# Hi-FT/ERD

Measured on AMD Instinct MI355X. Metric: images/sec GFL-R50 40+40 incre step @1333x800, higher is better.
Workload: dtype f32; 1 GPU; gfl_r50_fpn first_40_incre_last_40 ERD (BASELINE configs[1]), 1333x800 padded to 800x1344, fp32, procedural weights; batch_per_gpu=4, global_batch=4, parallelism=dp1

## Files before the change

### erd_amd/csrc/conv_mfma.hip

```cpp
#include <algorithm>
#include <type_traits>
#include "erd_common.h"
#include <stdlib.h>
#ifndef ERD_SGB
#define ERD_SGB 0
#endif

namespace {

typedef float f32x16 __attribute__((ext_vector_type(16)));
typedef __bf16 bf16x8 __attribute__((ext_vector_type(8)));
typedef __bf16 bf16x2v __attribute__((ext_vector_type(2)));
typedef float f32x2v __attribute__((ext_vector_type(2)));

__device__ __forceinline__ float pack_bf16(float a, float b) {
    const f32x2v v = {a, b};
    return __builtin_bit_cast(float, __builtin_convertvector(v, bf16x2v));
}

constexpr int NTHREADS = 256;

#ifdef ERD_IGEMM_TRACE
constexpr int IG_NS = 32;
__device__ unsigned long long g_igemm_trace[1024 * IG_NS];
// ... 1650 lines not shown
        int s = 0;
        for (; s + 3 < nsplit; s += 4) {
            const float4 v0 = *reinterpret_cast<const float4*>(part + (s + 0) * slab + o);
            const float4 v1 = *reinterpret_cast<const float4*>(part + (s + 1) * slab + o);
            const float4 v2 = *reinterpret_cast<const float4*>(part + (s + 2) * slab + o);
            const float4 v3 = *reinterpret_cast<const float4*>(part + (s + 3) * slab + o);
            g.x += (v0.x + v1.x) + (v2.x + v3.x); g.y += (v0.y + v1.y) + (v2.y + v3.y);
            g.z += (v0.z + v1.z) + (v2.z + v3.z); g.w += (v0.w + v1.w) + (v2.w + v3.w);
        }
        for (; s < nsplit; ++s) {
            const float4 v = *reinterpret_cast<const float4*>(part + s * slab + o);
            g.x += v.x; g.y += v.y; g.z += v.z; g.w += v.w;
        }
        if (rowdot) {
            const float4 ww = *reinterpret_cast<const float4*>(w + o);
            dot = ww.x * g.x + ww.y * g.y + ww.z * g.z + ww.w * g.w;
        }
        float4 o4 = make_float4(rs * g.x, rs * g.y, rs * g.z, rs * g.w);
        if (accumulate) {
            const float4 old = *reinterpret_cast<const float4*>(dW + o);
            o4.x += old.x; o4.y += old.y; o4.z += old.z; o4.w += old.w;
        }
        *reinterpret_cast<float4*>(dW + o) = o4;
    }
    if (rowdot) {
        __shared__ float red[4];
        dot = erd::wave_sum(dot);
        if ((threadIdx.x & 63) == 0) red[threadIdx.x >> 6] = dot;
        __syncthreads();
        if (threadIdx.x == 0) atomicAdd(rowdot + co, red[0] + red[1] + red[2] + red[3]);
    }
}

template <typename OutT>
__global__ __launch_bounds__(256) void weight_transpose_kernel(const float* __restrict__ w,
                                                                const float* __restrict__ rowscale,
                                                                OutT* __restrict__ dst, int Cout, int ntaps, int Cin,
                                                                int flip) {
    __shared__ float tile[32][33];
    const int t = blockIdx.z;
    const int td = flip ? ntaps - 1 - t : t;
    const int ci0 = blockIdx.x * 32, co0 = blockIdx.y * 32;
    const int tx = threadIdx.x & 31, ty = threadIdx.x >> 5;
    for (int r = ty; r < 32; r += 8) {
        const int co = co0 + r, ci = ci0 + tx;
        float v = 0.f;
        if (co < Cout && ci < Cin) v = w[((int64_t)co * ntaps + t) * Cin + ci] * (rowscale ? rowscale[co] : 1.f);
        tile[r][tx] = v;
    }
    __syncthreads();
    for (int r = ty; r < 32; r += 8) {
        const int ci = ci0 + r, co = co0 + tx;
        if (co < Cout && ci < Cin) dst[((int64_t)ci * ntaps + td) * Cout + co] = (OutT)tile[tx][r];
    }
}

using erd::limbs3;

__global__ __launch_bounds__(256) void split3_kernel(const float* __restrict__ src, unsigned short* __restrict__ dst, int64_t n) {
    const int64_t i = blockIdx.x * 256ll + threadIdx.x;
    if (i >= n) return;
    unsigned short h, m, l;
    limbs3(src[i], h, m, l);
    dst[i] = h;
    dst[n + i] = m;
    dst[2 * n + i] = l;
}

__global__ __launch_bounds__(256) void weight_transpose_x3_kernel(const float* __restrict__ w, const float* __restrict__ rowscale,
                                                                   unsigned short* __restrict__ dst, int Cout, int ntaps, int Cin,
                                                                   int flip) {
    __shared__ float tile[32][33];
    const int t = blockIdx.z;
    const int td = flip ? ntaps - 1 - t : t;
    const int ci0 = blockIdx.x * 32, co0 = blockIdx.y * 32;
    const int tx = threadIdx.x & 31, ty = threadIdx.x >> 5;
    for (int r = ty; r < 32; r += 8) {
        const int co = co0 + r, ci = ci0 + tx;
        float v = 0.f;
        if (co < Cout && ci < Cin) v = w[((int64_t)co * ntaps + t) * Cin + ci] * (rowscale ? rowscale[co] : 1.f);
        tile[r][tx] = v;
    }
    __syncthreads();
    const int64_t plane = (int64_t)Cin * ntaps * Cout;
    for (int r = ty; r < 32; r += 8) {
        const int ci = ci0 + r, co = co0 + tx;
        if (co < Cout && ci < Cin) {
            unsigned short h, m, l;
            limbs3(tile[tx][r], h, m, l);
            const int64_t o = ((int64_t)ci * ntaps + td) * Cout + co;
            dst[o] = h;
            dst[plane + o] = m;
            dst[2 * plane + o] = l;
        }
    }
}

int num_cus() {
    static int n = 0;
    if (n == 0) {
        int dev = 0;
        hipDeviceProp_t prop;
        if (hipGetDevice(&dev) == hipSuccess && hipGetDeviceProperties(&prop, dev) == hipSuccess)
            n = prop.multiProcessorCount;
        if (n <= 0) n = 256;
    }
    return n;
}

struct IgemmShape { int64_t mtiles; bool seg_taps; };

int igemm_plan(const erd_conv_desc* d, const IgemmShape& sh, int tiles, int nkt, int BKT, int MINW, bool BF, SkWs& ws) {
    const int slots = MINW * erd::usable_cus(num_cus());
    int G = tiles;
    ws = SkWs{nullptr, nullptr, xcd_order_enabled(), 0};
    const size_t slab_bytes = (size_t)2 * 4 * num_cus() * 128 * 128 * sizeof(float);
    const size_t need = slab_bytes + (size_t)tiles * sizeof(int);
    const bool ragged = tiles < 8 * slots && (tiles % slots) != 0;
    const bool sk_pays = BF ? tiles * 2 <= slots : true;
    static const int min_slices = getenv("ERD_SK_MIN_SLICES") ? atoi(getenv("ERD_SK_MIN_SLICES")) : 8;
    const int64_t units = (int64_t)tiles * nkt;
    const bool tiny = units < slots && min_slices > 0 && nkt >= 2 * min_slices && !BF;
    if (sh.seg_taps) ws.xcd_order = 0;
    static const int sk_min_k = getenv("ERD_SK_MIN_K") ? atoi(getenv("ERD_SK_MIN_K")) : 512;
    if (d->sk_ws && d->sk_ws_bytes >= need && ragged && sk_pays && !sh.seg_taps && nkt * BKT >= sk_min_k && (units >= slots || tiny)) {
        G = (int)std::min<int64_t>(slots, min_slices > 0 ? std::max<int64_t>(tiles, units / min_slices) : slots);
        ws.slabs = reinterpret_cast<float*>(d->sk_ws);
        ws.cnt = reinterpret_cast<int*>(reinterpret_cast<char*>(d->sk_ws) + slab_bytes);
// ... 231 lines not shown
    if (rowdot && !(accumulate & 2)) (void)hipMemsetAsync(rowdot, 0, sizeof(float) * Cout, (hipStream_t)stream);
    hipLaunchKernelGGL(wgrad_reduce_kernel, dim3(Cout, (K + 1023) / 1024), dim3(256), 0, (hipStream_t)stream, part,
                       nsplit, Cout, K, w, rowscale, dW, accumulate & 1, rowdot, erd_wgrad_reduce_groups{});
    return erd::check_launch("wgrad_reduce");
}

extern "C" int erd_wgrad_reduce_grouped(const float* part, int nsplit, int Cout, int K, const erd_wgrad_reduce_groups* groups,
                                        int accumulate, erd_stream_t stream) {
    ERD_REQUIRE(part && groups && nsplit >= 1 && Cout >= 1 && K >= 4 && K % 4 == 0, "wgrad_reduce_grouped: bad args");
    ERD_REQUIRE(groups->ngroups >= 1 && groups->ngroups <= ERD_MAX_GROUPS, "wgrad_reduce_grouped: ngroups=%d", groups->ngroups);
    for (int g = 0; g < groups->ngroups; ++g) {
        ERD_REQUIRE(groups->dW[g], "wgrad_reduce_grouped: group %d has no dW", g);
        ERD_REQUIRE(!groups->rowdot[g] || groups->w[g], "wgrad_reduce_grouped: rowdot of group %d needs w", g);
    }
    if (!(accumulate & 2))
        for (int g = 0; g < groups->ngroups; ++g)
            if (groups->rowdot[g]) (void)hipMemsetAsync(groups->rowdot[g], 0, sizeof(float) * Cout, (hipStream_t)stream);
    hipLaunchKernelGGL(wgrad_reduce_kernel, dim3(Cout, (K + 1023) / 1024, groups->ngroups), dim3(256), 0, (hipStream_t)stream, part,
                       nsplit, Cout, K, nullptr, nullptr, nullptr, accumulate & 1, nullptr, *groups);
    return erd::check_launch("wgrad_reduce_grouped");
}

extern "C" int erd_wgrad_reduce_rows(const float* part, int nsplit, int Cout_slab, int Cout, int K, float* dW,
                                     int accumulate, erd_stream_t stream) {
    ERD_REQUIRE(part && dW && nsplit >= 1 && K % 4 == 0 && Cout >= 1 && Cout <= Cout_slab, "wgrad_reduce_rows: bad args");
    hipLaunchKernelGGL(wgrad_reduce_kernel, dim3(Cout, (K + 1023) / 1024), dim3(256), 0, (hipStream_t)stream, part,
                       nsplit, Cout_slab, K, nullptr, nullptr, dW, accumulate & 1, nullptr, erd_wgrad_reduce_groups{});
    return erd::check_launch("wgrad_reduce_rows");
}

extern "C" int erd_weight_transpose(const float* w, const float* rowscale, float* dst, int Cout, int ntaps,
                                    int Cin, int flip, erd_stream_t stream) {
    ERD_REQUIRE(w && dst && Cout > 0 && Cin > 0 && ntaps > 0, "weight_transpose: bad args");
    hipLaunchKernelGGL(weight_transpose_kernel<float>, dim3((Cin + 31) / 32, (Cout + 31) / 32, ntaps), dim3(256), 0,
                       (hipStream_t)stream, w, rowscale, dst, Cout, ntaps, Cin, flip);
    return erd::check_launch("weight_transpose");
}

extern "C" int erd_split3(const float* src, void* dst, int64_t n, erd_stream_t stream) {
    ERD_REQUIRE(src && dst && n > 0, "split3: bad args");
    hipLaunchKernelGGL(split3_kernel, dim3((unsigned)((n + 255) / 256)), dim3(256), 0, (hipStream_t)stream, src,
                       reinterpret_cast<unsigned short*>(dst), n);
    return erd::check_launch("split3");
}

extern "C" int erd_weight_transpose_x3(const float* w, const float* rowscale, void* dst, int Cout, int ntaps, int Cin, int flip,
                                       erd_stream_t stream) {
    ERD_REQUIRE(w && dst && Cout > 0 && Cin > 0 && ntaps > 0, "weight_transpose_x3: bad args");
    hipLaunchKernelGGL(weight_transpose_x3_kernel, dim3((Cin + 31) / 32, (Cout + 31) / 32, ntaps), dim3(256), 0, (hipStream_t)stream, w,
                       rowscale, reinterpret_cast<unsigned short*>(dst), Cout, ntaps, Cin, flip);
    return erd::check_launch("weight_transpose_x3");
}

extern "C" int erd_weight_transpose_bf16(const float* w, const float* rowscale, void* dst, int Cout, int ntaps,
                                         int Cin, int flip, erd_stream_t stream) {
    ERD_REQUIRE(w && dst && Cout > 0 && Cin > 0 && ntaps > 0, "weight_transpose_bf16: bad args");
    hipLaunchKernelGGL(weight_transpose_kernel<__bf16>, dim3((Cin + 31) / 32, (Cout + 31) / 32, ntaps), dim3(256), 0,
                       (hipStream_t)stream, w, rowscale, reinterpret_cast<__bf16*>(dst), Cout, ntaps, Cin, flip);
    return erd::check_launch("weight_transpose_bf16");
}
```

### erd_amd/csrc/erd_common.h

```cpp
#pragma once
#include <hip/hip_runtime.h>
#include <stdint.h>
#include <stdio.h>
#include <stdarg.h>
#include "../../include/erd_hip.h"
#include "erd_probes.h"

namespace erd {

void set_error(const char* fmt, ...);
int usable_cus(int physical);

bool conv_thin_x3_ok(const erd_conv_desc* d);
int conv_thin_x3(const erd_conv_desc* d, hipStream_t st);
bool conv_thin_bf16_ok(const erd_conv_desc* d);
int conv_thin_bf16(const erd_conv_desc* d, hipStream_t st);

inline int check_launch(const char* what) {
    hipError_t e = hipGetLastError();
    if (e != hipSuccess) {
        set_error("%s: %s", what, hipGetErrorString(e));
        return (int)e;
    }
    return 0;
// ... 57 lines not shown
__device__ __forceinline__ uint2 pack4_bf16(float4 v) { return make_uint2(pack2_bf16(v.x, v.y), pack2_bf16(v.z, v.w)); }

template <typename T>
__device__ __forceinline__ T* uniform_ptr(T* p) {
    const unsigned long long v = reinterpret_cast<unsigned long long>(p);
    const unsigned lo = __builtin_amdgcn_readfirstlane((unsigned)v), hi = __builtin_amdgcn_readfirstlane((unsigned)(v >> 32));
    return reinterpret_cast<T*>(((unsigned long long)hi << 32) | lo);
}
__device__ __forceinline__ int uniform_int(int v) { return __builtin_amdgcn_readfirstlane(v); }

__device__ __forceinline__ int xcd_contiguous(unsigned block, int grid) {
    const int q = grid >> 3, r = grid & 7, xcd = block & 7, idx = block >> 3;
    return (xcd < r ? xcd * (q + 1) : r * (q + 1) + (xcd - r) * q) + idx;
}

__device__ __forceinline__ float scalar_op(float v) {
    asm("" : "+v"(v));
    return v;
}
__device__ __forceinline__ void limbs3_pair(float x0, float x1, unsigned& hi, unsigned& mid, unsigned& lo) {
    hi = pack2_bf16(x0, x1);
    const float r0 = scalar_op(x0 - bf16_lo(hi)), r1 = scalar_op(x1 - bf16_hi(hi));
    mid = pack2_bf16(r0, r1);
    lo = pack2_bf16(scalar_op(r0 - bf16_lo(mid)), scalar_op(r1 - bf16_hi(mid)));
}
__device__ __forceinline__ void limbs3(float x, unsigned short& hi, unsigned short& mid, unsigned short& lo) {
    unsigned h, m, l;
    limbs3_pair(x, 0.f, h, m, l);
    hi = (unsigned short)(h & 0xffffu);
    mid = (unsigned short)(m & 0xffffu);
    lo = (unsigned short)(l & 0xffffu);
}

__device__ __forceinline__ void wino_x3_weight_item(const float* __restrict__ w, unsigned short* __restrict__ U3, int Cout, int Cin,
                                                    int flip, int co, int ci) {
    float g[3][3];
#pragma unroll
    for (int a = 0; a < 3; ++a)
#pragma unroll
        for (int b = 0; b < 3; ++b)
            g[a][b] = co < Cout ? w[((int64_t)co * 9 + (flip ? 8 - (a * 3 + b) : a * 3 + b)) * Cin + ci] : 0.f;
    float t[4][3];
#pragma unroll
    for (int b = 0; b < 3; ++b) {
        t[0][b] = g[0][b];
        t[1][b] = 0.5f * (g[0][b] + g[1][b] + g[2][b]);
        t[2][b] = 0.5f * (g[0][b] - g[1][b] + g[2][b]);
        t[3][b] = g[2][b];
    }
    const int nks = Cin / 16, ncb32 = (Cout + 31) / 32;
    const int64_t per_xl = (int64_t)ncb32 * nks * 512;
    const int64_t base = (((int64_t)(co / 32) * nks + ci / 16) * 64 + ((ci % 16) / 8) * 32 + (co % 32)) * 8 + (ci % 8);
#pragma unroll
    for (int i = 0; i < 4; ++i) {
        const float u[4] = {t[i][0], 0.5f * (t[i][0] + t[i][1] + t[i][2]), 0.5f * (t[i][0] - t[i][1] + t[i][2]), t[i][2]};
#pragma unroll
        for (int j = 0; j < 4; ++j) {
            unsigned short hi, mid, lo;
            limbs3(u[j], hi, mid, lo);
            const int64_t o = (int64_t)((i * 4 + j) * 3) * per_xl + base;
            U3[o] = hi;
            U3[o + per_xl] = mid;
            U3[o + 2 * per_xl] = lo;
        }
    }
}

struct bf16s { unsigned short bits; };
__device__ __forceinline__ float4 ld4(const float* p) { return *reinterpret_cast<const float4*>(p); }
__device__ __forceinline__ float4 ld4(const bf16s* p) { return unpack4_bf16(*reinterpret_cast<const uint2*>(p)); }
__device__ __forceinline__ void st4(float* p, float4 v) { *reinterpret_cast<float4*>(p) = v; }
__device__ __forceinline__ void st4(bf16s* p, float4 v) { *reinterpret_cast<uint2*>(p) = pack4_bf16(v); }
__device__ __forceinline__ float ld1(const float* p) { return *p; }
__device__ __forceinline__ float ld1(const bf16s* p) { return __uint_as_float((unsigned)p->bits << 16); }
__device__ __forceinline__ void st1(float* p, float v) { *p = v; }
__device__ __forceinline__ void st1(bf16s* p, float v) { p->bits = (unsigned short)(pack2_bf16(v, 0.f) & 0xffffu); }

}
```

### erd_amd/csrc/prep.hip

```cpp
#include "erd_common.h"

namespace {

__device__ __forceinline__ void transpose_block(const erd_weight_prep_item& it, int local, float (*tile)[33]) {
    const int nbx = (it.Cin + 31) / 32, nby = (it.Cout + 31) / 32;
    const int bx = local % nbx, by = (local / nbx) % nby, t = local / (nbx * nby);
    const int td = it.flip ? it.ntaps - 1 - t : t;
    const int ci0 = bx * 32, co0 = by * 32;
    const int tx = threadIdx.x & 31, ty = threadIdx.x >> 5;
    const float* __restrict__ w = it.w;
    for (int r = ty; r < 32; r += 8) {
        const int co = co0 + r, ci = ci0 + tx;
        float v = 0.f;
        if (co < it.Cout && ci < it.Cin) v = w[((int64_t)co * it.ntaps + t) * it.Cin + ci] * (it.rowscale ? it.rowscale[co] : 1.f);
        tile[r][tx] = v;
    }
    __syncthreads();
    for (int r = ty; r < 32; r += 8) {
        const int ci = ci0 + r, co = co0 + tx;
        if (co < it.Cout && ci < it.Cin) {
            const int64_t o = ((int64_t)ci * it.ntaps + td) * it.Cout + co;
            if (it.kind == 1) reinterpret_cast<__bf16*>(it.dst)[o] = (__bf16)tile[tx][r];
            else reinterpret_cast<float*>(it.dst)[o] = tile[tx][r];
        }
    }
}

__device__ __forceinline__ void wino_block(const erd_weight_prep_item& it, int local) {
    const int Cout = it.Cout, Cin = it.Cin, flip = it.flip;
    const float* __restrict__ w = it.w;
    float* __restrict__ U = reinterpret_cast<float*>(it.dst);
    const int cop = (Cout + 15) / 16 * 16;
    const int64_t idx = local * 256ll + threadIdx.x;
    if (idx >= (int64_t)cop * Cin) return;
    const int co = (int)(idx / Cin), ci = (int)(idx % Cin);
    float g[3][3];
#pragma unroll
    for (int a = 0; a < 3; ++a)
#pragma unroll
        for (int b = 0; b < 3; ++b)
            g[a][b] = co < Cout ? w[((int64_t)co * 9 + (flip ? 8 - (a * 3 + b) : a * 3 + b)) * Cin + ci] : 0.f;
    float t[4][3];
#pragma unroll
    for (int b = 0; b < 3; ++b) {
        t[0][b] = g[0][b];
        t[1][b] = 0.5f * (g[0][b] + g[1][b] + g[2][b]);
        t[2][b] = 0.5f * (g[0][b] - g[1][b] + g[2][b]);
        t[3][b] = g[2][b];
    }
    const int nks = Cin / 16;
    const int64_t per_xi = (int64_t)(cop / 16) * nks * 256;
    const int64_t base = (((int64_t)(co / 16) * nks + ci / 16) * 4 + (ci % 16) / 4) * 64 + (co % 16) * 4 + (ci % 4);
#pragma unroll
    for (int i = 0; i < 4; ++i) {
        const float u0 = t[i][0], u1 = 0.5f * (t[i][0] + t[i][1] + t[i][2]), u2 = 0.5f * (t[i][0] - t[i][1] + t[i][2]),
                    u3 = t[i][2];
        U[(i * 4 + 0) * per_xi + base] = u0;
        U[(i * 4 + 1) * per_xi + base] = u1;
        U[(i * 4 + 2) * per_xi + base] = u2;
        U[(i * 4 + 3) * per_xi + base] = u3;
    }
}

__device__ __forceinline__ void split3_block(const erd_weight_prep_item& it, int local) {
    const int64_t n = (int64_t)it.Cout * it.ntaps * it.Cin;
    const int64_t i = local * 256ll + threadIdx.x;
    if (i >= n) return;
    unsigned short h, m, l;
    erd::limbs3(it.w[i], h, m, l);
    unsigned short* d = reinterpret_cast<unsigned short*>(it.dst);
    d[i] = h;
    d[n + i] = m;
    d[2 * n + i] = l;
}

__device__ __forceinline__ void wino_x3_block(const erd_weight_prep_item& it, int local) {
    const int cop = (it.Cout + 31) / 32 * 32;
    const int64_t idx = local * 256ll + threadIdx.x;
    if (idx >= (int64_t)cop * it.Cin) return;
    erd::wino_x3_weight_item(it.w, reinterpret_cast<unsigned short*>(it.dst), it.Cout, it.Cin, it.flip, (int)(idx / it.Cin), (int)(idx % it.Cin));
}

__global__ __launch_bounds__(256) void weight_prep_kernel(const erd_weight_prep_item* __restrict__ items, int nitems) {
    __shared__ float tile[32][33];
    __shared__ int s_item;
    if (threadIdx.x == 0) {
        int lo = 0, hi = nitems - 1;
        while (lo < hi) {
            const int mid = (lo + hi + 1) >> 1;
            if (items[mid].block0 <= (int)blockIdx.x) lo = mid; else hi = mid - 1;
        }
        s_item = lo;
    }
    __syncthreads();
    const erd_weight_prep_item it = items[s_item];
    const int local = (int)blockIdx.x - it.block0;
    if (it.kind == 2) wino_block(it, local);
    else if (it.kind == 3) split3_block(it, local);
    else if (it.kind == 4) wino_x3_block(it, local);
    else transpose_block(it, local, tile);
}

}

extern "C" int erd_weight_prep_blocks(int kind, int Cout, int ntaps, int Cin) {
    if (kind == 2) return (int)(((int64_t)((Cout + 15) / 16 * 16) * Cin + 255) / 256);
    if (kind == 3) return (int)(((int64_t)Cout * ntaps * Cin + 255) / 256);
    if (kind == 4) return (int)(((int64_t)((Cout + 31) / 32 * 32) * Cin + 255) / 256);
    return ((Cin + 31) / 32) * ((Cout + 31) / 32) * ntaps;
}

extern "C" int erd_weight_prep_batch(const erd_weight_prep_item* items_dev, int nitems, int total_blocks, erd_stream_t stream) {
    ERD_REQUIRE(items_dev && nitems >= 0 && total_blocks >= 0, "weight_prep_batch: bad args");
    if (nitems == 0 || total_blocks == 0) return 0;
    hipLaunchKernelGGL(weight_prep_kernel, dim3((unsigned)total_blocks), dim3(256), 0, (hipStream_t)stream, items_dev, nitems);
    return erd::check_launch("weight_prep_batch");
}
```

### erd_amd/csrc/winograd.hip

```cpp
#include "erd_common.h"
#include <type_traits>
#include <stdlib.h>
#include <algorithm>

namespace {

typedef float f32x4 __attribute__((ext_vector_type(4)));
typedef unsigned int u32x4 __attribute__((ext_vector_type(4)));
constexpr unsigned OOBV = 0x80000000u;

__device__ __forceinline__ float4 buf_load16_s(__amdgpu_buffer_rsrc_t r, unsigned voff, unsigned soff) {
    const u32x4 v = __builtin_amdgcn_raw_buffer_load_b128(r, voff, soff, 0);
    return make_float4(__uint_as_float(v.x), __uint_as_float(v.y), __uint_as_float(v.z), __uint_as_float(v.w));
}

constexpr int KS = 16;
constexpr int BN = 64;
constexpr int BNP = 128;
constexpr int RCS = 6;
#ifndef ERD_WINO_NCH
#define ERD_WINO_NCH 4
#endif
constexpr int NCH = ERD_WINO_NCH;
constexpr int MAXPIX = 64 * NCH;
constexpr int RAW_LDS_F4 = MAXPIX * RCS;
constexpr int V_F4 = 16 * 32 * (KS / 4);
constexpr int MAXREG = 16;

__device__ __forceinline__ float4 f4add(float4 a, float4 b) { return make_float4(a.x + b.x, a.y + b.y, a.z + b.z, a.w + b.w); }
__device__ __forceinline__ float4 f4sub(float4 a, float4 b) { return make_float4(a.x - b.x, a.y - b.y, a.z - b.z, a.w - b.w); }
__device__ __forceinline__ int vswz2(int row, int c) { return c ^ ((0 - (row >> 2)) & 3); }

#ifdef ERD_WINO_TRACE
__device__ unsigned long long g_wino_trace[256 * 8];
__device__ unsigned long long g_wino_trace_p[256 * 16];
#define ERD_T0(v) const unsigned long long v = __builtin_amdgcn_s_memtime()
#define ERD_TACC(acc, v) acc += __builtin_amdgcn_s_memtime() - v
#else
#define ERD_T0(v)
#define ERD_TACC(acc, v)
#endif

__global__ __launch_bounds__(256) void wino_weight_kernel(const float* __restrict__ w, float* __restrict__ U, int Cout,
                                                           int Cin, int flip) {
    const int cop = (Cout + 15) / 16 * 16;
    const int64_t idx = blockIdx.x * 256ll + threadIdx.x;
    if (idx >= (int64_t)cop * Cin) return;
    const int co = (int)(idx / Cin), ci = (int)(idx % Cin);
    float g[3][3];
#pragma unroll
    for (int a = 0; a < 3; ++a)
#pragma unroll
        for (int b = 0; b < 3; ++b)
            g[a][b] = co < Cout ? w[((int64_t)co * 9 + (flip ? 8 - (a * 3 + b) : a * 3 + b)) * Cin + ci] : 0.f;
    float t[4][3];
#pragma unroll
    for (int b = 0; b < 3; ++b) {
        t[0][b] = g[0][b];
        t[1][b] = 0.5f * (g[0][b] + g[1][b] + g[2][b]);
        t[2][b] = 0.5f * (g[0][b] - g[1][b] + g[2][b]);
        t[3][b] = g[2][b];
    }
    const int nks = Cin / 16;
    const int64_t per_xi = (int64_t)(cop / 16) * nks * 256;
    const int64_t base = (((int64_t)(co / 16) * nks + ci / 16) * 4 + (ci % 16) / 4) * 64 + (co % 16) * 4 + (ci % 4);
#pragma unroll
    for (int i = 0; i < 4; ++i) {
        const float u0 = t[i][0], u1 = 0.5f * (t[i][0] + t[i][1] + t[i][2]), u2 = 0.5f * (t[i][0] - t[i][1] + t[i][2]),
                    u3 = t[i][2];
        U[(i * 4 + 0) * per_xi + base] = u0;
        U[(i * 4 + 1) * per_xi + base] = u1;
        U[(i * 4 + 2) * per_xi + base] = u2;
        U[(i * 4 + 3) * per_xi + base] = u3;
    }
}


struct WinoSeg {
    const float* in;
    float* out;
    const float* res;
    const float* mask;
    int N, H, W;
    int64_t in_nstride, out_nstride;
};
struct WinoRegion {
    int seg, ty0, tx0, nby, nbx, lbw;
    int block0;
    int ty1, tx1;
};
struct WinoDesc {
    int nseg, nreg;
    WinoSeg seg[ERD_MAX_SEG];
    WinoRegion reg[MAXREG];
    const float* U;
    const void* U3;
    int Cin, Cout;
    const float* scale;
    const float* shift;
    int relu;
    float* colsum;
    int colsum_copies;
    int blocks_per_nb;
    int nitems;
    int* sched;
    float* gn_part;
};
// ... 1338 lines not shown

__global__ __launch_bounds__(512) void wino_gn_finalize_kernel(const WinoDesc p, float* __restrict__ mean_rstd, float eps) {
    const int G = p.Cout >> 3;
    const int nb = blockIdx.x, s = blockIdx.y, n = blockIdx.z;
    if (n >= p.seg[s].N) return;
    const int q = threadIdx.x & 31, il = threadIdx.x >> 5;
    double acc = 0.0;
    for (int r = 0; r < p.nreg; ++r) {
        const WinoRegion& rg = p.reg[r];
        if (rg.seg != s) continue;
        const int per_img = rg.nby * rg.nbx;
        const int64_t it0 = (int64_t)nb * p.blocks_per_nb + rg.block0 + (int64_t)n * per_img;
        for (int b = il; b < per_img; b += 16) acc += (double)p.gn_part[(it0 + b) * 32 + q];
    }
    __shared__ double red[16][32];
    red[il][q] = acc;
    __syncthreads();
    if (threadIdx.x < 16) {
        const int gi = threadIdx.x;
        double s1 = 0.0, s2 = 0.0;
        for (int l = 0; l < 16; ++l) { s1 += red[l][2 * gi]; s2 += red[l][2 * gi + 1]; }
        const double m = (double)p.seg[s].H * p.seg[s].W * 8.0;
        const double mean = s1 / m;
        double var = s2 / m - mean * mean;
        if (var < 0) var = 0;
        const int64_t i = ((int64_t)n * p.nseg + s) * G + nb * 16 + gi;
        mean_rstd[i * 2] = (float)mean;
        mean_rstd[i * 2 + 1] = (float)(1.0 / sqrt(var + (double)eps));
    }
}

__global__ __launch_bounds__(256) void wino_weight_x3_kernel(const float* __restrict__ w, unsigned short* __restrict__ U3, int Cout,
                                                              int Cin, int flip) {
    const int cop = (Cout + 31) / 32 * 32;
    const int64_t idx = blockIdx.x * 256ll + threadIdx.x;
    if (idx >= (int64_t)cop * Cin) return;
    erd::wino_x3_weight_item(w, U3, Cout, Cin, flip, (int)(idx / Cin), (int)(idx % Cin));
}

}

extern "C" int erd_wino_weights(const float* w_ohwi, float* U, int Cout, int Cin, int flip, erd_stream_t stream) {
    ERD_REQUIRE(w_ohwi && U && Cout > 0 && Cin > 0 && Cin % KS == 0, "wino_weights: Cin=%d must be a multiple of %d", Cin, KS);
    const int64_t n = (int64_t)((Cout + 15) / 16 * 16) * Cin;
    hipLaunchKernelGGL(wino_weight_kernel, dim3((unsigned)((n + 255) / 256)), dim3(256), 0, (hipStream_t)stream, w_ohwi, U,
                       Cout, Cin, flip);
    return erd::check_launch("wino_weights");
}

#ifdef ERD_WINO_TRACE
extern "C" int erd_wino_trace(unsigned long long* out) {
    (void)hipDeviceSynchronize();
    return (int)hipMemcpyFromSymbol(out, HIP_SYMBOL(g_wino_trace), sizeof(g_wino_trace));
}
extern "C" int erd_wino_trace_p(unsigned long long* out) {
    (void)hipDeviceSynchronize();
    return (int)hipMemcpyFromSymbol(out, HIP_SYMBOL(g_wino_trace_p), sizeof(g_wino_trace_p));
}
#endif

extern "C" size_t erd_wino_weights_elems(int Cout, int Cin) { return (size_t)16 * ((Cout + 15) / 16 * 16) * Cin; }

namespace {
int wino_plan(WinoDesc& d, const erd_conv_seg* segs, int nseg, bool x3, int Cout, int& ncu, bool& phased) {
    ERD_REQUIRE(segs && nseg >= 1 && nseg <= ERD_MAX_SEG, "wino: bad args");
    d.nseg = nseg;
    static const int shapes = getenv("ERD_WINO_SHAPES") ? atoi(getenv("ERD_WINO_SHAPES")) : 1;
    int blocks = 0, nreg = 0;
    auto add_region = [&](int s, int N, int ty0, int tx0, int nby, int nbx, int lbw, int ty1, int tx1) {
        if (nby <= 0 || nbx <= 0) return;
        WinoRegion& r = d.reg[nreg++];
        r.seg = s; r.ty0 = ty0; r.tx0 = tx0; r.nby = nby; r.nbx = nbx; r.lbw = lbw; r.ty1 = ty1; r.tx1 = tx1;
        r.block0 = blocks;
        blocks += N * nby * nbx;
    };
    for (int s = 0; s < nseg; ++s) {
        const erd_conv_seg& g = segs[s];
        ERD_REQUIRE(g.in && g.out && g.IH == g.OH && g.IW == g.OW, "wino: segment %d is not a stride-1 same-size map", s);
// ... 97 lines not shown
    if (U3) {
        const size_t lds = (size_t)2 * RAW_LDS_F4 * sizeof(float4) + 2 * VX_B + 4 * 2 * XCH_B + 64 + 2048 + 16;
        static bool attr3_done = false;
        if (!attr3_done) {
            (void)hipFuncSetAttribute(reinterpret_cast<const void*>(wino_x3_kernel), hipFuncAttributeMaxDynamicSharedMemorySize, (int)lds);
            attr3_done = true;
        }
        hipLaunchKernelGGL(wino_x3_kernel, dim3((unsigned)grid), dim3(512), lds, stream, d);
        return erd::check_launch("wino_conv3x3_x3");
    }
    const size_t lds = (size_t)2 * (RAW_LDS_F4 + V_F4) * sizeof(float4) + 2048 + 16;
    static bool attr_done = false;
    if (!attr_done) {
        (void)hipFuncSetAttribute(reinterpret_cast<const void*>(wino_conv_kernel), hipFuncAttributeMaxDynamicSharedMemorySize,
                                  (int)lds);
        attr_done = true;
    }
    hipLaunchKernelGGL(wino_conv_kernel, dim3((unsigned)grid), dim3(512), lds, stream, d);
    return erd::check_launch("wino_conv3x3");
}
}

extern "C" int erd_wino_conv3x3(const erd_conv_seg* segs, int nseg, const float* U, int Cin, int Cout,
                                const float* scale, const float* shift, int relu, float* colsum, int colsum_copies,
                                int* sched, erd_stream_t stream) {
    ERD_REQUIRE(U, "wino: null U");
    return wino_launch(segs, nseg, U, nullptr, Cin, Cout, scale, shift, relu, colsum, colsum_copies, sched, (hipStream_t)stream);
}

extern "C" size_t erd_wino_weights_x3_elems(int Cout, int Cin) { return (size_t)16 * 3 * ((Cout + 31) / 32 * 32) * Cin; }

extern "C" int erd_wino_weights_x3(const float* w_ohwi, void* U3, int Cout, int Cin, int flip, erd_stream_t stream) {
    ERD_REQUIRE(w_ohwi && U3 && Cout > 0 && Cin > 0 && Cin % KS == 0, "wino_weights_x3: Cin=%d must be a multiple of %d", Cin, KS);
    const int64_t n = (int64_t)((Cout + 31) / 32 * 32) * Cin;
    hipLaunchKernelGGL(wino_weight_x3_kernel, dim3((unsigned)((n + 255) / 256)), dim3(256), 0, (hipStream_t)stream, w_ohwi,
                       reinterpret_cast<unsigned short*>(U3), Cout, Cin, flip);
    return erd::check_launch("wino_weights_x3");
}

extern "C" int erd_wino_x3_couts_per_item(const erd_conv_seg* segs, int nseg, int Cout) {
    WinoDesc d;
    int ncu = 0;
    bool phased = false;
    if (wino_plan(d, segs, nseg, true, Cout, ncu, phased)) return -1;
    return phased ? BNP : BN;
}

extern "C" int erd_wino_conv3x3_x3(const erd_conv_seg* segs, int nseg, const void* U3, int Cin, int Cout,
                                   const float* scale, const float* shift, int relu, float* colsum, int colsum_copies,
                                   int* sched, erd_stream_t stream) {
    ERD_REQUIRE(U3, "wino_x3: null U3");
    return wino_launch(segs, nseg, nullptr, U3, Cin, Cout, scale, shift, relu, colsum, colsum_copies, sched, (hipStream_t)stream);
}

extern "C" int erd_wino_conv3x3_x3_gn(const erd_conv_seg* segs, int nseg, const void* U3, int Cin, int Cout, const float* scale,
                                      const float* shift, int relu, int* sched, float* gn_part, size_t gn_part_bytes,
                                      erd_stream_t stream) {
    ERD_REQUIRE(U3 && gn_part, "wino_x3_gn: null U3 / gn_part");
    return wino_launch(segs, nseg, nullptr, U3, Cin, Cout, scale, shift, relu, nullptr, 0, sched, (hipStream_t)stream, gn_part, gn_part_bytes);
}

extern "C" int erd_wino_gn_finalize(const erd_conv_seg* segs, int nseg, int Cout, const float* gn_part, float* mean_rstd, float eps,
                                    erd_stream_t stream) {
    ERD_REQUIRE(segs && gn_part && mean_rstd && Cout % BNP == 0, "wino_gn_finalize: bad args");
    WinoDesc d;
    int ncu = 0, nmax = 0;
    bool phased = false;
    if (const int rc = wino_plan(d, segs, nseg, true, Cout, ncu, phased)) return rc;
// ... 17 lines not shown
```

Baseline: 131.9 images/sec.

## Vectorize weight-prep kernels: 64x64 transpose tiles, octet split3, per-wave Winograd units

Reworks the per-step weight preparation kernels (transpose to fp32/bf16/3-limb, split3, Winograd fp32 and x3 weight transforms) to use vectorized float4/uint4 loads and stores. The transpose tile grows from 32x32 to 64x64 with 4-wide accesses, split3 processes 8 elements per thread, and Winograd weight transforms assign one wave per transform row with coalesced 16-byte stores instead of scattered scalar writes. The target is the many small memory-bound prep launches each step. The cost is more code paths with alignment fallbacks and a new alignment requirement on U.

```diff
diff --git a/erd_amd/csrc/conv_mfma.hip b/erd_amd/csrc/conv_mfma.hip
--- a/erd_amd/csrc/conv_mfma.hip
+++ b/erd_amd/csrc/conv_mfma.hip
@@ -1706,68 +1706,16 @@
     }
 }
 
-template <typename OutT>
-__global__ __launch_bounds__(256) void weight_transpose_kernel(const float* __restrict__ w,
-                                                                const float* __restrict__ rowscale,
-                                                                OutT* __restrict__ dst, int Cout, int ntaps, int Cin,
-                                                                int flip) {
-    __shared__ float tile[32][33];
-    const int t = blockIdx.z;
-    const int td = flip ? ntaps - 1 - t : t;
-    const int ci0 = blockIdx.x * 32, co0 = blockIdx.y * 32;
-    const int tx = threadIdx.x & 31, ty = threadIdx.x >> 5;
-    for (int r = ty; r < 32; r += 8) {
-        const int co = co0 + r, ci = ci0 + tx;
-        float v = 0.f;
-        if (co < Cout && ci < Cin) v = w[((int64_t)co * ntaps + t) * Cin + ci] * (rowscale ? rowscale[co] : 1.f);
-        tile[r][tx] = v;
-    }
-    __syncthreads();
-    for (int r = ty; r < 32; r += 8) {
-        const int ci = ci0 + r, co = co0 + tx;
-        if (co < Cout && ci < Cin) dst[((int64_t)ci * ntaps + td) * Cout + co] = (OutT)tile[tx][r];
-    }
-}
-
-using erd::limbs3;
+template <int FORM>
+__global__ __launch_bounds__(256) void weight_transpose_kernel(const float* __restrict__ w, const float* __restrict__ rowscale,
+                                                                void* __restrict__ dst, int Cout, int ntaps, int Cin, int flip) {
+    __shared__ float tile[erd::WT_TILE][erd::WT_TILE + 1];
+    erd::weight_transpose_tile<FORM>(w, rowscale, dst, Cout, ntaps, Cin, flip, (int)blockIdx.x * erd::WT_TILE, (int)blockIdx.y * erd::WT_TILE,
+                                     (int)blockIdx.z, tile);
+}
 
 __global__ __launch_bounds__(256) void split3_kernel(const float* __restrict__ src, unsigned short* __restrict__ dst, int64_t n) {
-    const int64_t i = blockIdx.x * 256ll + threadIdx.x;
-    if (i >= n) return;
-    unsigned short h, m, l;
-    limbs3(src[i], h, m, l);
-    dst[i] = h;
-    dst[n + i] = m;
-    dst[2 * n + i] = l;
-}
-
-__global__ __launch_bounds__(256) void weight_transpose_x3_kernel(const float* __restrict__ w, const float* __restrict__ rowscale,
-                                                                   unsigned short* __restrict__ dst, int Cout, int ntaps, int Cin,
-                                                                   int flip) {
-    __shared__ float tile[32][33];
-    const int t = blockIdx.z;
-    const int td = flip ? ntaps - 1 - t : t;
-    const int ci0 = blockIdx.x * 32, co0 = blockIdx.y * 32;
-    const int tx = threadIdx.x & 31, ty = threadIdx.x >> 5;
-    for (int r = ty; r < 32; r += 8) {
-        const int co = co0 + r, ci = ci0 + tx;
-        float v = 0.f;
-        if (co < Cout && ci < Cin) v = w[((int64_t)co * ntaps + t) * Cin + ci] * (rowscale ? rowscale[co] : 1.f);
-        tile[r][tx] = v;
-    }
-    __syncthreads();
-    const int64_t plane = (int64_t)Cin * ntaps * Cout;
-    for (int r = ty; r < 32; r += 8) {
-        const int ci = ci0 + r, co = co0 + tx;
-        if (co < Cout && ci < Cin) {
-            unsigned short h, m, l;
-            limbs3(tile[tx][r], h, m, l);
-            const int64_t o = ((int64_t)ci * ntaps + td) * Cout + co;
-            dst[o] = h;
-            dst[plane + o] = m;
-            dst[2 * plane + o] = l;
-        }
-    }
+    erd::split3_octet(src, dst, n, (blockIdx.x * 256ll + threadIdx.x) * 8);
 }
 
 int num_cus() {
@@ -2065,14 +2013,14 @@
 extern "C" int erd_weight_transpose(const float* w, const float* rowscale, float* dst, int Cout, int ntaps,
                                     int Cin, int flip, erd_stream_t stream) {
     ERD_REQUIRE(w && dst && Cout > 0 && Cin > 0 && ntaps > 0, "weight_transpose: bad args");
-    hipLaunchKernelGGL(weight_transpose_kernel<float>, dim3((Cin + 31) / 32, (Cout + 31) / 32, ntaps), dim3(256), 0,
-                       (hipStream_t)stream, w, rowscale, dst, Cout, ntaps, Cin, flip);
+    hipLaunchKernelGGL(weight_transpose_kernel<0>, dim3((Cin + erd::WT_TILE - 1) / erd::WT_TILE, (Cout + erd::WT_TILE - 1) / erd::WT_TILE, ntaps),
+                       dim3(256), 0, (hipStream_t)stream, w, rowscale, (void*)dst, Cout, ntaps, Cin, flip);
     return erd::check_launch("weight_transpose");
 }
 
 extern "C" int erd_split3(const float* src, void* dst, int64_t n, erd_stream_t stream) {
     ERD_REQUIRE(src && dst && n > 0, "split3: bad args");
-    hipLaunchKernelGGL(split3_kernel, dim3((unsigned)((n + 255) / 256)), dim3(256), 0, (hipStream_t)stream, src,
+    hipLaunchKernelGGL(split3_kernel, dim3((unsigned)((n + 2047) / 2048)), dim3(256), 0, (hipStream_t)stream, src,
                        reinterpret_cast<unsigned short*>(dst), n);
     return erd::check_launch("split3");
 }
@@ -2080,15 +2028,15 @@
 extern "C" int erd_weight_transpose_x3(const float* w, const float* rowscale, void* dst, int Cout, int ntaps, int Cin, int flip,
                                        erd_stream_t stream) {
     ERD_REQUIRE(w && dst && Cout > 0 && Cin > 0 && ntaps > 0, "weight_transpose_x3: bad args");
-    hipLaunchKernelGGL(weight_transpose_x3_kernel, dim3((Cin + 31) / 32, (Cout + 31) / 32, ntaps), dim3(256), 0, (hipStream_t)stream, w,
-                       rowscale, reinterpret_cast<unsigned short*>(dst), Cout, ntaps, Cin, flip);
+    hipLaunchKernelGGL(weight_transpose_kernel<2>, dim3((Cin + erd::WT_TILE - 1) / erd::WT_TILE, (Cout + erd::WT_TILE - 1) / erd::WT_TILE, ntaps),
+                       dim3(256), 0, (hipStream_t)stream, w, rowscale, dst, Cout, ntaps, Cin, flip);
     return erd::check_launch("weight_transpose_x3");
 }
 
 extern "C" int erd_weight_transpose_bf16(const float* w, const float* rowscale, void* dst, int Cout, int ntaps,
                                          int Cin, int flip, erd_stream_t stream) {
     ERD_REQUIRE(w && dst && Cout > 0 && Cin > 0 && ntaps > 0, "weight_transpose_bf16: bad args");
-    hipLaunchKernelGGL(weight_transpose_kernel<__bf16>, dim3((Cin + 31) / 32, (Cout + 31) / 32, ntaps), dim3(256), 0,
-                       (hipStream_t)stream, w, rowscale, reinterpret_cast<__bf16*>(dst), Cout, ntaps, Cin, flip);
+    hipLaunchKernelGGL(weight_transpose_kernel<1>, dim3((Cin + erd::WT_TILE - 1) / erd::WT_TILE, (Cout + erd::WT_TILE - 1) / erd::WT_TILE, ntaps),
+                       dim3(256), 0, (hipStream_t)stream, w, rowscale, dst, Cout, ntaps, Cin, flip);
     return erd::check_launch("weight_transpose_bf16");
 }
diff --git a/erd_amd/csrc/erd_common.h b/erd_amd/csrc/erd_common.h
--- a/erd_amd/csrc/erd_common.h
+++ b/erd_amd/csrc/erd_common.h
@@ -113,36 +113,202 @@
     lo = (unsigned short)(l & 0xffffu);
 }
 
-__device__ __forceinline__ void wino_x3_weight_item(const float* __restrict__ w, unsigned short* __restrict__ U3, int Cout, int Cin,
-                                                    int flip, int co, int ci) {
-    float g[3][3];
-#pragma unroll
-    for (int a = 0; a < 3; ++a)
-#pragma unroll
-        for (int b = 0; b < 3; ++b)
-            g[a][b] = co < Cout ? w[((int64_t)co * 9 + (flip ? 8 - (a * 3 + b) : a * 3 + b)) * Cin + ci] : 0.f;
-    float t[4][3];
-#pragma unroll
-    for (int b = 0; b < 3; ++b) {
-        t[0][b] = g[0][b];
-        t[1][b] = 0.5f * (g[0][b] + g[1][b] + g[2][b]);
-        t[2][b] = 0.5f * (g[0][b] - g[1][b] + g[2][b]);
-        t[3][b] = g[2][b];
-    }
+__host__ __device__ __forceinline__ bool aligned16(const void* p) { return (reinterpret_cast<uintptr_t>(p) & 15) == 0; }
+template <int N>
+__device__ __forceinline__ void ldn(const float* __restrict__ p, bool vec, float (&v)[N]) {
+    if (vec) {
+#pragma unroll
+        for (int q = 0; q < N / 4; ++q) {
+            const float4 x = reinterpret_cast<const float4*>(p)[q];
+            v[q * 4] = x.x; v[q * 4 + 1] = x.y; v[q * 4 + 2] = x.z; v[q * 4 + 3] = x.w;
+        }
+    } else {
+#pragma unroll
+        for (int q = 0; q < N; ++q) v[q] = p[q];
+    }
+}
+__device__ __forceinline__ void limbs3_octet(const float (&x)[8], uint4& hi, uint4& mid, uint4& lo) {
+    limbs3_pair(x[0], x[1], hi.x, mid.x, lo.x);
+    limbs3_pair(x[2], x[3], hi.y, mid.y, lo.y);
+    limbs3_pair(x[4], x[5], hi.z, mid.z, lo.z);
+    limbs3_pair(x[6], x[7], hi.w, mid.w, lo.w);
+}
+
+template <int NC>
+__device__ __forceinline__ void wino_weight_row(const float* __restrict__ w, int Cout, int Cin, int flip, int co, int ci, int i,
+                                                float (&u)[4][NC]) {
+    const bool vec = aligned16(w);
+    const float* __restrict__ row = w + (int64_t)co * 9 * Cin + ci;
+    auto tap = [&](int k, float (&g)[NC]) {
+        if (co < Cout) {
+            ldn<NC>(row + (int64_t)(flip ? 8 - k : k) * Cin, vec, g);
+        } else {
+#pragma unroll
+            for (int c = 0; c < NC; ++c) g[c] = 0.f;
+        }
+    };
+    float t[3][NC];
+    if (i == 0 || i == 3) {
+#pragma unroll
+        for (int b = 0; b < 3; ++b) tap((i == 0 ? 0 : 6) + b, t[b]);
+    } else {
+#pragma unroll
+        for (int b = 0; b < 3; ++b) {
+            float g0[NC], g1[NC], g2[NC];
+            tap(b, g0);
+            tap(3 + b, g1);
+            tap(6 + b, g2);
+#pragma unroll
+            for (int c = 0; c < NC; ++c) t[b][c] = i == 1 ? 0.5f * (g0[c] + g1[c] + g2[c]) : 0.5f * (g0[c] - g1[c] + g2[c]);
+        }
+    }
+#pragma unroll
+    for (int c = 0; c < NC; ++c) {
+        u[0][c] = t[0][c];
+        u[1][c] = 0.5f * (t[0][c] + t[1][c] + t[2][c]);
+        u[2][c] = 0.5f * (t[0][c] - t[1][c] + t[2][c]);
+        u[3][c] = t[2][c];
+    }
+}
+
+__device__ __forceinline__ void wino_weight_unit(const float* __restrict__ w, float* __restrict__ U, int Cout, int Cin, int flip,
+                                                 int unit, int i, int lane) {
+    const int nks = Cin / 16, ncb = (Cout + 15) / 16;
+    const int co = (unit / nks) * 16 + (lane & 15), ci = (unit % nks) * 16 + (lane >> 4) * 4;
+    float u[4][4];
+    wino_weight_row<4>(w, Cout, Cin, flip, co, ci, i, u);
+    const int64_t per_xi = (int64_t)ncb * nks * 256;
+    float* __restrict__ o = U + ((int64_t)unit * 64 + lane) * 4 + (int64_t)(i * 4) * per_xi;
+#pragma unroll
+    for (int j = 0; j < 4; ++j) *reinterpret_cast<float4*>(o + j * per_xi) = make_float4(u[j][0], u[j][1], u[j][2], u[j][3]);
+}
+
+__device__ __forceinline__ void wino_x3_weight_unit(const float* __restrict__ w, unsigned short* __restrict__ U3, int Cout, int Cin,
+                                                    int flip, int unit, int i, int lane) {
     const int nks = Cin / 16, ncb32 = (Cout + 31) / 32;
+    const int co = (unit / nks) * 32 + (lane & 31), ci = (unit % nks) * 16 + (lane >> 5) * 8;
+    float u[4][8];
+    wino_weight_row<8>(w, Cout, Cin, flip, co, ci, i, u);
     const int64_t per_xl = (int64_t)ncb32 * nks * 512;
-    const int64_t base = (((int64_t)(co / 32) * nks + ci / 16) * 64 + ((ci % 16) / 8) * 32 + (co % 32)) * 8 + (ci % 8);
-#pragma unroll
-    for (int i = 0; i < 4; ++i) {
-        const float u[4] = {t[i][0], 0.5f * (t[i][0] + t[i][1] + t[i][2]), 0.5f * (t[i][0] - t[i][1] + t[i][2]), t[i][2]};
-#pragma unroll
-        for (int j = 0; j < 4; ++j) {
-            unsigned short hi, mid, lo;
-            limbs3(u[j], hi, mid, lo);
-            const int64_t o = (int64_t)((i * 4 + j) * 3) * per_xl + base;
-            U3[o] = hi;
-            U3[o + per_xl] = mid;
-            U3[o + 2 * per_xl] = lo;
+    unsigned short* __restrict__ o = U3 + ((int64_t)unit * 64 + lane) * 8 + (int64_t)(i * 12) * per_xl;
+#pragma unroll
+    for (int j = 0; j < 4; ++j) {
+        uint4 hi, mid, lo;
+        limbs3_octet(u[j], hi, mid, lo);
+        *reinterpret_cast<uint4*>(o + (int64_t)(j * 3) * per_xl) = hi;
+        *reinterpret_cast<uint4*>(o + (int64_t)(j * 3 + 1) * per_xl) = mid;
+        *reinterpret_cast<uint4*>(o + (int64_t)(j * 3 + 2) * per_xl) = lo;
+    }
+}
+
+__device__ __forceinline__ void split3_octet(const float* __restrict__ src, unsigned short* __restrict__ dst, int64_t n, int64_t i0) {
+    if (i0 >= n) return;
+    if (i0 + 8 <= n) {
+        float x[8];
+        ldn<8>(src + i0, aligned16(src + i0), x);
+        uint4 l[3];
+        limbs3_octet(x, l[0], l[1], l[2]);
+#pragma unroll
+        for (int p = 0; p < 3; ++p) {
+            unsigned short* d = dst + p * n + i0;
+            if (aligned16(d)) {
+                *reinterpret_cast<uint4*>(d) = l[p];
+            } else {
+                const unsigned wd[4] = {l[p].x, l[p].y, l[p].z, l[p].w};
+#pragma unroll
+                for (int q = 0; q < 8; ++q) d[q] = (unsigned short)(wd[q >> 1] >> ((q & 1) * 16));
+            }
+        }
+        return;
+    }
+    for (int64_t i = i0; i < n; ++i) {
+        unsigned short h, m, l;
+        limbs3(src[i], h, m, l);
+        dst[i] = h;
+        dst[n + i] = m;
+        dst[2 * n + i] = l;
+    }
+}
+
+constexpr int WT_TILE = 64;
+template <int FORM>
+__device__ __forceinline__ void weight_transpose_tile(const float* __restrict__ w, const float* __restrict__ rowscale, void* __restrict__ dstv,
+                                                      int Cout, int ntaps, int Cin, int flip, int ci0, int co0, int t,
+                                                      float (*tile)[WT_TILE + 1]) {
+    const int tid = threadIdx.x;
+    const int td = flip ? ntaps - 1 - t : t;
+    {
+        const bool vec = (Cin & 3) == 0 && aligned16(w);
+        const int c = (tid & 15) * 4, ci = ci0 + c;
+#pragma unroll
+        for (int p = 0; p < 4; ++p) {
+            const int r = p * 16 + (tid >> 4), co = co0 + r;
+            float v[4] = {0.f, 0.f, 0.f, 0.f};
+            if (co < Cout && ci < Cin) {
+                const float* __restrict__ s = w + ((int64_t)co * ntaps + t) * Cin + ci;
+                const float rs = rowscale ? rowscale[co] : 1.f;
+                if (vec) {
+                    ldn<4>(s, true, v);
+                } else {
+#pragma unroll
+                    for (int j = 0; j < 4; ++j)
+                        if (ci + j < Cin) v[j] = s[j];
+                }
+#pragma unroll
+                for (int j = 0; j < 4; ++j) v[j] *= rs;
+            }
+#pragma unroll
+            for (int j = 0; j < 4; ++j) tile[r][c + j] = v[j];
+        }
+    }
+    __syncthreads();
+    const int64_t plane = (int64_t)Cin * ntaps * Cout;
+    if constexpr (FORM == 0) {
+        float* __restrict__ dst = reinterpret_cast<float*>(dstv);
+        const bool vec = (Cout & 3) == 0 && aligned16(dst);
+        const int c = (tid & 15) * 4, co = co0 + c;
+#pragma unroll
+        for (int p = 0; p < 4; ++p) {
+            const int r = p * 16 + (tid >> 4), ci = ci0 + r;
+            if (ci >= Cin || co >= Cout) continue;
+            float* __restrict__ d = dst + ((int64_t)ci * ntaps + td) * Cout + co;
+            if (vec) {
+                *reinterpret_cast<float4*>(d) = make_float4(tile[c][r], tile[c + 1][r], tile[c + 2][r], tile[c + 3][r]);
+            } else {
+#pragma unroll
+                for (int j = 0; j < 4; ++j)
+                    if (co + j < Cout) d[j] = tile[c + j][r];
+            }
+        }
+    } else {
+        unsigned short* __restrict__ dst = reinterpret_cast<unsigned short*>(dstv);
+        const bool vec = (Cout & 7) == 0 && aligned16(dst);
+        const int c = (tid & 7) * 8, co = co0 + c;
+#pragma unroll
+        for (int p = 0; p < 2; ++p) {
+            const int r = p * 32 + (tid >> 3), ci = ci0 + r;
+            if (ci >= Cin || co >= Cout) continue;
+            unsigned short* __restrict__ d = dst + ((int64_t)ci * ntaps + td) * Cout + co;
+            float x[8];
+#pragma unroll
+            for (int j = 0; j < 8; ++j) x[j] = tile[c + j][r];
+            uint4 l[3];
+            if constexpr (FORM == 1) {
+                l[0] = make_uint4(pack2_bf16(x[0], x[1]), pack2_bf16(x[2], x[3]), pack2_bf16(x[4], x[5]), pack2_bf16(x[6], x[7]));
+            } else {
+                limbs3_octet(x, l[0], l[1], l[2]);
+            }
+#pragma unroll
+            for (int q = 0; q < (FORM == 1 ? 1 : 3); ++q) {
+                if (vec) {
+                    *reinterpret_cast<uint4*>(d + q * plane) = l[q];
+                } else {
+                    const unsigned wd[4] = {l[q].x, l[q].y, l[q].z, l[q].w};
+#pragma unroll
+                    for (int j = 0; j < 8; ++j)
+                        if (co + j < Cout) d[q * plane + j] = (unsigned short)(wd[j >> 1] >> ((j & 1) * 16));
+                }
+            }
         }
     }
 }
diff --git a/erd_amd/csrc/prep.hip b/erd_amd/csrc/prep.hip
--- a/erd_amd/csrc/prep.hip
+++ b/erd_amd/csrc/prep.hip
@@ -2,87 +2,8 @@
 
 namespace {
 
-__device__ __forceinline__ void transpose_block(const erd_weight_prep_item& it, int local, float (*tile)[33]) {
-    const int nbx = (it.Cin + 31) / 32, nby = (it.Cout + 31) / 32;
-    const int bx = local % nbx, by = (local / nbx) % nby, t = local / (nbx * nby);
-    const int td = it.flip ? it.ntaps - 1 - t : t;
-    const int ci0 = bx * 32, co0 = by * 32;
-    const int tx = threadIdx.x & 31, ty = threadIdx.x >> 5;
-    const float* __restrict__ w = it.w;
-    for (int r = ty; r < 32; r += 8) {
-        const int co = co0 + r, ci = ci0 + tx;
-        float v = 0.f;
-        if (co < it.Cout && ci < it.Cin) v = w[((int64_t)co * it.ntaps + t) * it.Cin + ci] * (it.rowscale ? it.rowscale[co] : 1.f);
-        tile[r][tx] = v;
-    }
-    __syncthreads();
-    for (int r = ty; r < 32; r += 8) {
-        const int ci = ci0 + r, co = co0 + tx;
-        if (co < it.Cout && ci < it.Cin) {
-            const int64_t o = ((int64_t)ci * it.ntaps + td) * it.Cout + co;
-            if (it.kind == 1) reinterpret_cast<__bf16*>(it.dst)[o] = (__bf16)tile[tx][r];
-            else reinterpret_cast<float*>(it.dst)[o] = tile[tx][r];
-        }
-    }
-}
-
-__device__ __forceinline__ void wino_block(const erd_weight_prep_item& it, int local) {
-    const int Cout = it.Cout, Cin = it.Cin, flip = it.flip;
-    const float* __restrict__ w = it.w;
-    float* __restrict__ U = reinterpret_cast<float*>(it.dst);
-    const int cop = (Cout + 15) / 16 * 16;
-    const int64_t idx = local * 256ll + threadIdx.x;
-    if (idx >= (int64_t)cop * Cin) return;
-    const int co = (int)(idx / Cin), ci = (int)(idx % Cin);
-    float g[3][3];
-#pragma unroll
-    for (int a = 0; a < 3; ++a)
-#pragma unroll
-        for (int b = 0; b < 3; ++b)
-            g[a][b] = co < Cout ? w[((int64_t)co * 9 + (flip ? 8 - (a * 3 + b) : a * 3 + b)) * Cin + ci] : 0.f;
-    float t[4][3];
-#pragma unroll
-    for (int b = 0; b < 3; ++b) {
-        t[0][b] = g[0][b];
-        t[1][b] = 0.5f * (g[0][b] + g[1][b] + g[2][b]);
-        t[2][b] = 0.5f * (g[0][b] - g[1][b] + g[2][b]);
-        t[3][b] = g[2][b];
-    }
-    const int nks = Cin / 16;
-    const int64_t per_xi = (int64_t)(cop / 16) * nks * 256;
-    const int64_t base = (((int64_t)(co / 16) * nks + ci / 16) * 4 + (ci % 16) / 4) * 64 + (co % 16) * 4 + (ci % 4);
-#pragma unroll
-    for (int i = 0; i < 4; ++i) {
-        const float u0 = t[i][0], u1 = 0.5f * (t[i][0] + t[i][1] + t[i][2]), u2 = 0.5f * (t[i][0] - t[i][1] + t[i][2]),
-                    u3 = t[i][2];
-        U[(i * 4 + 0) * per_xi + base] = u0;
-        U[(i * 4 + 1) * per_xi + base] = u1;
-        U[(i * 4 + 2) * per_xi + base] = u2;
-        U[(i * 4 + 3) * per_xi + base] = u3;
-    }
-}
-
-__device__ __forceinline__ void split3_block(const erd_weight_prep_item& it, int local) {
-    const int64_t n = (int64_t)it.Cout * it.ntaps * it.Cin;
-    const int64_t i = local * 256ll + threadIdx.x;
-    if (i >= n) return;
-    unsigned short h, m, l;
-    erd::limbs3(it.w[i], h, m, l);
-    unsigned short* d = reinterpret_cast<unsigned short*>(it.dst);
-    d[i] = h;
-    d[n + i] = m;
-    d[2 * n + i] = l;
-}
-
-__device__ __forceinline__ void wino_x3_block(const erd_weight_prep_item& it, int local) {
-    const int cop = (it.Cout + 31) / 32 * 32;
-    const int64_t idx = local * 256ll + threadIdx.x;
-    if (idx >= (int64_t)cop * it.Cin) return;
-    erd::wino_x3_weight_item(it.w, reinterpret_cast<unsigned short*>(it.dst), it.Cout, it.Cin, it.flip, (int)(idx / it.Cin), (int)(idx % it.Cin));
-}
-
 __global__ __launch_bounds__(256) void weight_prep_kernel(const erd_weight_prep_item* __restrict__ items, int nitems) {
-    __shared__ float tile[32][33];
+    __shared__ float tile[erd::WT_TILE][erd::WT_TILE + 1];
     __shared__ int s_item;
     if (threadIdx.x == 0) {
         int lo = 0, hi = nitems - 1;
@@ -95,19 +16,29 @@
     __syncthreads();
     const erd_weight_prep_item it = items[s_item];
     const int local = (int)blockIdx.x - it.block0;
-    if (it.kind == 2) wino_block(it, local);
-    else if (it.kind == 3) split3_block(it, local);
-    else if (it.kind == 4) wino_x3_block(it, local);
-    else transpose_block(it, local, tile);
+    const int wave = threadIdx.x >> 6, lane = threadIdx.x & 63;
+    if (it.kind == 2) {
+        erd::wino_weight_unit(it.w, reinterpret_cast<float*>(it.dst), it.Cout, it.Cin, it.flip, local, wave, lane);
+    } else if (it.kind == 3) {
+        erd::split3_octet(it.w, reinterpret_cast<unsigned short*>(it.dst), (int64_t)it.Cout * it.ntaps * it.Cin,
+                          (local * 256ll + threadIdx.x) * 8);
+    } else if (it.kind == 4) {
+        erd::wino_x3_weight_unit(it.w, reinterpret_cast<unsigned short*>(it.dst), it.Cout, it.Cin, it.flip, local, wave, lane);
+    } else {
+        const int nbx = (it.Cin + erd::WT_TILE - 1) / erd::WT_TILE, nby = (it.Cout + erd::WT_TILE - 1) / erd::WT_TILE;
+        const int ci0 = (local % nbx) * erd::WT_TILE, co0 = ((local / nbx) % nby) * erd::WT_TILE, t = local / (nbx * nby);
+        if (it.kind == 1) erd::weight_transpose_tile<1>(it.w, it.rowscale, it.dst, it.Cout, it.ntaps, it.Cin, it.flip, ci0, co0, t, tile);
+        else erd::weight_transpose_tile<0>(it.w, it.rowscale, it.dst, it.Cout, it.ntaps, it.Cin, it.flip, ci0, co0, t, tile);
+    }
 }
 
 }
 
 extern "C" int erd_weight_prep_blocks(int kind, int Cout, int ntaps, int Cin) {
-    if (kind == 2) return (int)(((int64_t)((Cout + 15) / 16 * 16) * Cin + 255) / 256);
-    if (kind == 3) return (int)(((int64_t)Cout * ntaps * Cin + 255) / 256);
-    if (kind == 4) return (int)(((int64_t)((Cout + 31) / 32 * 32) * Cin + 255) / 256);
-    return ((Cin + 31) / 32) * ((Cout + 31) / 32) * ntaps;
+    if (kind == 2) return ((Cout + 15) / 16) * (Cin / 16);
+    if (kind == 3) return (int)(((int64_t)Cout * ntaps * Cin + 2047) / 2048);
+    if (kind == 4) return ((Cout + 31) / 32) * (Cin / 16);
+    return ((Cin + erd::WT_TILE - 1) / erd::WT_TILE) * ((Cout + erd::WT_TILE - 1) / erd::WT_TILE) * ntaps;
 }
 
 extern "C" int erd_weight_prep_batch(const erd_weight_prep_item* items_dev, int nitems, int total_blocks, erd_stream_t stream) {
diff --git a/erd_amd/csrc/winograd.hip b/erd_amd/csrc/winograd.hip
--- a/erd_amd/csrc/winograd.hip
+++ b/erd_amd/csrc/winograd.hip
@@ -43,36 +43,7 @@
 
 __global__ __launch_bounds__(256) void wino_weight_kernel(const float* __restrict__ w, float* __restrict__ U, int Cout,
                                                            int Cin, int flip) {
-    const int cop = (Cout + 15) / 16 * 16;
-    const int64_t idx = blockIdx.x * 256ll + threadIdx.x;
-    if (idx >= (int64_t)cop * Cin) return;
-    const int co = (int)(idx / Cin), ci = (int)(idx % Cin);
-    float g[3][3];
-#pragma unroll
-    for (int a = 0; a < 3; ++a)
-#pragma unroll
-        for (int b = 0; b < 3; ++b)
-            g[a][b] = co < Cout ? w[((int64_t)co * 9 + (flip ? 8 - (a * 3 + b) : a * 3 + b)) * Cin + ci] : 0.f;
-    float t[4][3];
-#pragma unroll
-    for (int b = 0; b < 3; ++b) {
-        t[0][b] = g[0][b];
-        t[1][b] = 0.5f * (g[0][b] + g[1][b] + g[2][b]);
-        t[2][b] = 0.5f * (g[0][b] - g[1][b] + g[2][b]);
-        t[3][b] = g[2][b];
-    }
-    const int nks = Cin / 16;
-    const int64_t per_xi = (int64_t)(cop / 16) * nks * 256;
-    const int64_t base = (((int64_t)(co / 16) * nks + ci / 16) * 4 + (ci % 16) / 4) * 64 + (co % 16) * 4 + (ci % 4);
-#pragma unroll
-    for (int i = 0; i < 4; ++i) {
-        const float u0 = t[i][0], u1 = 0.5f * (t[i][0] + t[i][1] + t[i][2]), u2 = 0.5f * (t[i][0] - t[i][1] + t[i][2]),
-                    u3 = t[i][2];
-        U[(i * 4 + 0) * per_xi + base] = u0;
-        U[(i * 4 + 1) * per_xi + base] = u1;
-        U[(i * 4 + 2) * per_xi + base] = u2;
-        U[(i * 4 + 3) * per_xi + base] = u3;
-    }
+    erd::wino_weight_unit(w, U, Cout, Cin, flip, (int)blockIdx.x, (int)(threadIdx.x >> 6), (int)(threadIdx.x & 63));
 }
 
 
@@ -1477,18 +1448,16 @@
 
 __global__ __launch_bounds__(256) void wino_weight_x3_kernel(const float* __restrict__ w, unsigned short* __restrict__ U3, int Cout,
                                                               int Cin, int flip) {
-    const int cop = (Cout + 31) / 32 * 32;
-    const int64_t idx = blockIdx.x * 256ll + threadIdx.x;
-    if (idx >= (int64_t)cop * Cin) return;
-    erd::wino_x3_weight_item(w, U3, Cout, Cin, flip, (int)(idx / Cin), (int)(idx % Cin));
+    erd::wino_x3_weight_unit(w, U3, Cout, Cin, flip, (int)blockIdx.x, (int)(threadIdx.x >> 6), (int)(threadIdx.x & 63));
 }
 
 }
 
 extern "C" int erd_wino_weights(const float* w_ohwi, float* U, int Cout, int Cin, int flip, erd_stream_t stream) {
     ERD_REQUIRE(w_ohwi && U && Cout > 0 && Cin > 0 && Cin % KS == 0, "wino_weights: Cin=%d must be a multiple of %d", Cin, KS);
-    const int64_t n = (int64_t)((Cout + 15) / 16 * 16) * Cin;
-    hipLaunchKernelGGL(wino_weight_kernel, dim3((unsigned)((n + 255) / 256)), dim3(256), 0, (hipStream_t)stream, w_ohwi, U,
+    ERD_REQUIRE(erd::aligned16(U), "wino_weights: U must be 16-byte aligned");
+    const int units = (Cout + 15) / 16 * (Cin / 16);
+    hipLaunchKernelGGL(wino_weight_kernel, dim3((unsigned)units), dim3(256), 0, (hipStream_t)stream, w_ohwi, U,
                        Cout, Cin, flip);
     return erd::check_launch("wino_weights");
 }
@@ -1652,8 +1621,9 @@
 
 extern "C" int erd_wino_weights_x3(const float* w_ohwi, void* U3, int Cout, int Cin, int flip, erd_stream_t stream) {
     ERD_REQUIRE(w_ohwi && U3 && Cout > 0 && Cin > 0 && Cin % KS == 0, "wino_weights_x3: Cin=%d must be a multiple of %d", Cin, KS);
-    const int64_t n = (int64_t)((Cout + 31) / 32 * 32) * Cin;
-    hipLaunchKernelGGL(wino_weight_x3_kernel, dim3((unsigned)((n + 255) / 256)), dim3(256), 0, (hipStream_t)stream, w_ohwi,
+    ERD_REQUIRE(erd::aligned16(U3), "wino_weights_x3: U3 must be 16-byte aligned");
+    const int units = (Cout + 31) / 32 * (Cin / 16);
+    hipLaunchKernelGGL(wino_weight_x3_kernel, dim3((unsigned)units), dim3(256), 0, (hipStream_t)stream, w_ohwi,
                        reinterpret_cast<unsigned short*>(U3), Cout, Cin, flip);
     return erd::check_launch("wino_weights_x3");
 }
```

Result: no change. 132.4 images/sec (median of 6 runs) (+0.4%).
